# romanwerpachowski/ML

Measured on NVIDIA B200. Metric: em_point_components_per_second, higher is better.
Workload: dtype f64

## Files before the change

### ml_b200/csrc/context.cu

```cuda
#include <dlfcn.h>

#include <algorithm>
#include <cmath>
#include <cstdlib>
#include <cstring>
#include <mutex>
#include <random>
#include <string>
#include <thread>
#include <type_traits>
#include <vector>

#include "internal.h"

namespace mlb {

static thread_local std::string g_last_error = "";

void set_error(const char* fmt, ...)
{
    char buf[1024];
    va_list ap;
    va_start(ap, fmt);
    vsnprintf(buf, sizeof(buf), fmt, ap);
// ... 210 lines not shown
        sum += ms;
    }
    if (total_ms) *total_ms = sum;
    if (launches) *launches = static_cast<int64_t>(used / 2);
    return MLB_OK;
}

void KernelTimer::destroy()
{
    for (cudaEvent_t e : events)
        if (e) cudaEventDestroy(e);
    events.clear();
    used = 0;
}

Layout Layout::make(int64_t n_total)
{
    Layout lay;
    lay.n_total = n_total;
    int64_t c = n_total / (8 * kSmCount * 6);
    c = (c + 127) / 128 * 128;
    c = std::max<int64_t>(128, std::min<int64_t>(2048, c));
    if (const char* env = std::getenv("MLB200_CHUNK")) {
        const long v = std::atol(env);
        if (v >= 128 && v <= 4096 && v % 128 == 0) c = v;
    }
    lay.chunk = static_cast<int>(c);
    lay.n_chunks = (n_total + c - 1) / c;
    for (int v = 0; v <= kVirtualShards; ++v) lay.vshard_chunk[v] = lay.n_chunks * v / kVirtualShards;
    return lay;
}


struct VshardRanges {
    int64_t lo[kVirtualShards];
    int64_t hi[kVirtualShards];
};

__global__ void reduce_partials_kernel(const double* __restrict__ partials, VshardRanges r, int s, double* __restrict__ out)
{
    __shared__ double lanes[8][33];
    const int e = blockIdx.x * 32 + threadIdx.x;
    const int v = blockIdx.y, ty = threadIdx.y;
    double a0 = 0, a1 = 0, a2 = 0, a3 = 0;
    if (e < s) {
        const int64_t hi = r.hi[v];
        for (int64_t c = r.lo[v] + 4 * ty; c < hi; c += 32) {
            a0 += partials[c * s + e];
            if (c + 1 < hi) a1 += partials[(c + 1) * s + e];
            if (c + 2 < hi) a2 += partials[(c + 2) * s + e];
            if (c + 3 < hi) a3 += partials[(c + 3) * s + e];
        }
    }
    lanes[ty][threadIdx.x] = (a0 + a1) + (a2 + a3);
    __syncthreads();
    if (ty == 0 && e < s) {
        const int x = threadIdx.x;
        out[static_cast<int64_t>(v) * s + e] =
            ((lanes[0][x] + lanes[1][x]) + (lanes[2][x] + lanes[3][x])) + ((lanes[4][x] + lanes[5][x]) + (lanes[6][x] + lanes[7][x]));
    }
}

constexpr int kReduceGroup = 32;

__global__ void reduce_groups_kernel(const double* __restrict__ partials, VshardRanges r, int nv, int s, double* __restrict__ out)
{
    __shared__ double lanes[8][33];
    int group = blockIdx.y, v = 0;
    for (; v < nv; ++v) {
        const int ng = static_cast<int>((r.hi[v] - r.lo[v] + kReduceGroup - 1) / kReduceGroup);
        if (group < ng) break;
        group -= ng;
    }
    if (v == nv) return;
    const int64_t lo = r.lo[v] + static_cast<int64_t>(group) * kReduceGroup;
    const int64_t hi = min(lo + kReduceGroup, r.hi[v]);
    const int e = blockIdx.x * 32 + threadIdx.x, ty = threadIdx.y;
    double a0 = 0, a1 = 0, a2 = 0, a3 = 0;
    if (e < s) {
        const int64_t c = lo + 4 * ty;
        if (c < hi) a0 = partials[c * s + e];
        if (c + 1 < hi) a1 = partials[(c + 1) * s + e];
        if (c + 2 < hi) a2 = partials[(c + 2) * s + e];
        if (c + 3 < hi) a3 = partials[(c + 3) * s + e];
    }
    lanes[ty][threadIdx.x] = (a0 + a1) + (a2 + a3);
    __syncthreads();
    if (ty == 0 && e < s) {
        const int x = threadIdx.x;
        out[static_cast<int64_t>(blockIdx.y) * s + e] =
            ((lanes[0][x] + lanes[1][x]) + (lanes[2][x] + lanes[3][x])) + ((lanes[4][x] + lanes[5][x]) + (lanes[6][x] + lanes[7][x]));
    }
}

void ReduceScratch::release(mlb_ctx* ctx)
{
    for (size_t g = 0; g < ptr.size(); ++g)
        if (ptr[g]) {
            cudaSetDevice(ctx->gpus[g].device);
            cudaFreeAsync(ptr[g], ctx->gpus[g].stream);
        }
    ptr.clear();
    len.clear();
}

int reduce_and_exchange_units(mlb_data* data, const std::vector<double*>& partials, const std::vector<double*>& vsum, int s, ReduceScratch& scratch,
                              const int64_t* bounds)
{
    mlb_ctx* ctx = data->ctx;
    const int vpg = ctx->vshards_per_gpu();
    scratch.ptr.resize(ctx->gpus.size(), nullptr);
    scratch.len.resize(ctx->gpus.size(), 0);
    MLB_TRY(for_each_gpu(ctx, [&](int g, Gpu& gpu) -> int {
        const int64_t local_begin = bounds[gpu.rank * vpg];
        VshardRanges r, rg;
        int64_t total_groups = 0;
        for (int j = 0; j < vpg; ++j) {
            const int v = gpu.rank * vpg + j;
            r.lo[j] = bounds[v] - local_begin;
            r.hi[j] = bounds[v + 1] - local_begin;
            rg.lo[j] = total_groups;
            total_groups += (r.hi[j] - r.lo[j] + kReduceGroup - 1) / kReduceGroup;
            rg.hi[j] = total_groups;
        }
        double* out = vsum[g] + static_cast<int64_t>(gpu.rank) * vpg * s;
        if (bounds[kVirtualShards] <= 2 * kReduceGroup * kVirtualShards) {
            reduce_partials_kernel<<<dim3((s + 31) / 32, vpg), dim3(32, 8), 0, gpu.stream>>>(partials[g], r, s, out);
            MLB_CUDA(cudaGetLastError());
            return MLB_OK;
        }
        const size_t need = static_cast<size_t>(total_groups) * s;
        if (scratch.len[g] < need) {
            if (scratch.ptr[g]) {
                MLB_CUDA(cudaFreeAsync(scratch.ptr[g], gpu.stream));
                scratch.ptr[g] = nullptr;
                scratch.len[g] = 0;
            }
            MLB_CUDA(cudaMallocFromPoolAsync(&scratch.ptr[g], sizeof(double) * need, gpu.pool, gpu.stream));
            scratch.len[g] = need;
        }
        reduce_groups_kernel<<<dim3((s + 31) / 32, static_cast<unsigned>(total_groups)), dim3(32, 8), 0, gpu.stream>>>(partials[g], r, vpg, s, scratch.ptr[g]);
        MLB_CUDA(cudaGetLastError());
        reduce_partials_kernel<<<dim3((s + 31) / 32, vpg), dim3(32, 8), 0, gpu.stream>>>(scratch.ptr[g], rg, s, out);
        MLB_CUDA(cudaGetLastError());
        return MLB_OK;
    }));
    if (ctx->world > 1) {
        MLB_NCCL_API(api);
        MLB_NCCL(api, api->GroupStart());
        for (size_t g = 0; g < ctx->gpus.size(); ++g) {
            Gpu& gpu = ctx->gpus[g];
            const size_t count = static_cast<size_t>(vpg) * s;
            MLB_NCCL(api, api->AllGather(vsum[g] + static_cast<int64_t>(gpu.rank) * count, vsum[g], count, ncclDouble, gpu.comm, gpu.stream));
        }
        MLB_NCCL(api, api->GroupEnd());
    }
    return MLB_OK;
}

int reduce_and_exchange(mlb_data* data, const std::vector<double*>& partials, const std::vector<double*>& vsum, int s, ReduceScratch& scratch)
{
    return reduce_and_exchange_units(data, partials, vsum, s, scratch, data->lay.vshard_chunk);
}


__global__ void column_sum_kernel(const double* __restrict__ x, int64_t n_local, int d, int chunk, double* __restrict__ partials)
{
    extern __shared__ double sm[];
    const int64_t p0 = static_cast<int64_t>(blockIdx.x) * chunk;
    const int64_t p1 = min(p0 + chunk, n_local);
    const int lanes = blockDim.x / d;
    const int t = threadIdx.x;
    const int c = t % d, lane = t / d;
    double acc = 0;
    if (lane < lanes) {
        for (int64_t p = p0 + lane; p < p1; p += lanes) acc += x[p * d + c];
    }
    sm[t] = (lane < lanes) ? acc : 0.0;
    __syncthreads();
    if (t < d) {
        double s = 0;
        for (int l = 0; l < lanes; ++l) s += sm[l * d + t];
        partials[static_cast<int64_t>(blockIdx.x) * d + t] = s;
    }
}

static int compute_shift(mlb_data* data)
{
    mlb_ctx* ctx = data->ctx;
    const int d = data->d;
    std::vector<double*> partials(ctx->gpus.size(), nullptr), vsum(ctx->gpus.size(), nullptr);
    MLB_TRY(for_each_gpu(ctx, [&](int g, Gpu& gpu) -> int {
        DataShard& sh = data->shards[g];
        MLB_CUDA(cudaMallocFromPoolAsync(&partials[g], sizeof(double) * std::max<int64_t>(1, sh.n_chunks()) * d, gpu.pool, gpu.stream));
        MLB_CUDA(cudaMallocFromPoolAsync(&vsum[g], sizeof(double) * kVirtualShards * d, gpu.pool, gpu.stream));
// ... 645 lines not shown
```

### ml_b200/csrc/em.cu

```cuda
#include <algorithm>
#include <cmath>
#include <limits>

#include "em_direct.cuh"
#include "em_split.cuh"
#include "fastmath.cuh"
#include "internal.h"

namespace mlb {

constexpr int kTile = 64;
constexpr int kEmThreads = 128;
constexpr int kLogBatch = 16;

__host__ __device__ constexpr int em_ne_offdiag(int DP) { return 4 * (DP / 4) * (DP / 4 - 1) / 2; }
__host__ __device__ constexpr int em_ne(int DP) { return em_ne_offdiag(DP) + 2 * (DP / 4) + (DP / 4 + 1) / 2 + DP / 4; }
__host__ __device__ constexpr int em_estep_offdiag(int DP, int a, int mb)
{
    const int DQ = DP / 4, ma = a / 4, i = a % 4;
    int n = 0;
    for (int m = 0; m < ma; ++m) n += 4 * (DQ - 1 - m);
    return n + i * (DQ - 1 - ma) + (mb - ma - 1);
}
__host__ __device__ constexpr int em_fm_raw(int DP) { return 1 + DP + DP * (DP + 1) / 2; }
__host__ __device__ constexpr int em_nm(int DP) { return (em_fm_raw(DP) + 7) / 8; }
__host__ __device__ constexpr int em_sv(int DP, int KP) { return em_nm(DP) * 8 * KP + 8; }
__host__ __device__ constexpr int em_theta_len(int DP, int KP) { return em_ne(DP) * (KP / 8) * 32 + KP; }

constexpr size_t em_smem_bytes(int DP, int KP)
{
    return sizeof(double) * (em_theta_len(DP, KP) + 2 * kTile * (DP + 4) + kTile * (KP + 4) + 8 + DP + kExpTableSize);
}

struct EmArgs {
    const double* x;
    long long n_local;
    int d, k;
    const double* shift;
    const double* theta;
    const int2* feat_m;
    double* partials;
    int chunk;
    int n_chunks;
    unsigned* counter;
    const double* r_in;
    long long r_ld;
    double* r_out;
    long long r_out_ld;
    unsigned* labels_out;
    long long range_begin, range_count;
};

__device__ __forceinline__ long long min64(long long a, long long b) { return a < b ? a : b; }

__device__ __forceinline__ void dmma(double (&acc)[2], double a, double b)
{
    asm("mma.sync.aligned.m8n8k4.row.col.f64.f64.f64.f64 {%0,%1}, {%2}, {%3}, {%0,%1};" : "+d"(acc[0]), "+d"(acc[1]) : "d"(a), "d"(b));
}

template <int NT>
__device__ __forceinline__ void load_theta_frag(const double* thE, int j, int lane, double (&bf)[NT])
{
    if constexpr (NT == 1) {
        bf[0] = thE[j * 32 + lane];
    } else {
#pragma unroll
        for (int h = 0; h < NT / 2; ++h) {
            const double2 v = reinterpret_cast<const double2*>(thE)[(j * (NT / 2) + h) * 32 + lane];
            bf[2 * h] = v.x;
            bf[2 * h + 1] = v.y;
        }
    }
}

template <int DP, int KP, int MODE>
__global__ void __launch_bounds__(kEmThreads, (DP * KP <= 128 || MODE == 2) ? 4 : 2) em_kernel(const EmArgs p)
{
    constexpr int NT = KP / 8, DQ = DP / 4, NE = em_ne(DP), NM = em_nm(DP);
    constexpr int ZS = DP + 4, RS = KP + 4;
    constexpr int WN = (NM >= 8 || NT == 1) ? 1 : 2, WM = 4 / WN;
    constexpr int MW = (NM + WM - 1) / WM, NW = NT / WN;
    constexpr int SV = em_sv(DP, KP);
    constexpr int XR = kTile * DP / kEmThreads;

    extern __shared__ __align__(16) double sm[];
    double* thE = sm;
    double* cE = thE + NE * NT * 32;
    double* Zb = cE + KP;
    double* R = Zb + 2 * kTile * ZS;
    double* wl = R + kTile * RS;
    double* sh = wl + 8;
    double* etab = sh + DP;
    __shared__ int s_next;

    const int tid = threadIdx.x, lane = tid & 31, warp = tid >> 5, g = lane >> 2, c = lane & 3;
    const int d = p.d;

    if (MODE != 1)
        for (int i = tid; i < em_theta_len(DP, KP); i += kEmThreads) sm[i] = p.theta[i];
    for (int i = tid; i < 2 * kTile * ZS; i += kEmThreads) Zb[i] = 0.0;
    for (int i = tid; i < kTile * RS; i += kEmThreads) R[i] = 0.0;
    if (tid < DP) sh[tid] = tid < d ? p.shift[tid] : 0.0;
    load_exp_table(etab);

    const int wm = warp / WN, wn = warp % WN;
    int ia[MW], ib[MW];
    double sacc[MW][NW][2];
    if (MODE != 2) {
#pragma unroll
        for (int i = 0; i < MW; ++i) {
            const int mt = wm * MW + i;
            const int2 f = mt < NM ? p.feat_m[mt * 8 + g] : make_int2(DP + 1, DP + 1);
            ia[i] = f.x;
            ib[i] = f.y;
        }
    }

    double xr[XR];
    auto load_tile = [&](long long point0, int nvalid) {
        const double* xg = p.x + point0 * d;
        const int nel = nvalid * d;
#pragma unroll
        for (int r = 0; r < XR; ++r) {
            const int e = tid + kEmThreads * r;
            xr[r] = e < nel ? xg[e] : 0.0;
        }
    };
    auto store_tile = [&](double* Z, int nvalid) {
        const int nel = nvalid * d;
#pragma unroll
        for (int r = 0; r < XR; ++r) {
            const int e = tid + kEmThreads * r;
            if (e < kTile * d) {
                const int pt = (d == DP) ? e / DP : FastDiv(d).div(e);
                const int dm = e - pt * d;
                Z[pt * ZS + dm] = e < nel ? xr[r] - sh[dm] : 0.0;
            }
        }
        if (tid < kTile) Z[tid * ZS + DP] = tid < nvalid ? 1.0 : 0.0;
    };

    const long long work_begin = MODE == 2 ? p.range_begin : 0;
    const long long work_end = MODE == 2 ? p.range_begin + p.range_count : p.n_local;

    for (;;) {
        __syncthreads();
        if (tid == 0) s_next = static_cast<int>(atomicAdd(p.counter, 1u));
        __syncthreads();
        const int chunk = s_next;
        if (chunk >= p.n_chunks) break;
        const long long p_begin = work_begin + static_cast<long long>(chunk) * p.chunk;
        const long long p_end = min64(p_begin + p.chunk, work_end);
        const int ntiles = static_cast<int>((p_end - p_begin + kTile - 1) / kTile);

        if (MODE != 2) {
#pragma unroll
            for (int i = 0; i < MW; ++i)
#pragma unroll
                for (int nt = 0; nt < NW; ++nt) sacc[i][nt][0] = sacc[i][nt][1] = 0.0;
        }
        double ll_acc = 0.0, ll_prod = 1.0;

        load_tile(p_begin, static_cast<int>(min64(kTile, p_end - p_begin)));
        store_tile(Zb, static_cast<int>(min64(kTile, p_end - p_begin)));
        __syncthreads();

        for (int t = 0; t < ntiles; ++t) {
            double* Z = Zb + (t & 1) * kTile * ZS;
            const long long tile0 = p_begin + static_cast<long long>(t) * kTile;
            const int nvalid = static_cast<int>(min64(kTile, p_end - tile0));
            const int nvalid_next = t + 1 < ntiles ? static_cast<int>(min64(kTile, p_end - tile0 - kTile)) : 0;
            if (t + 1 < ntiles) load_tile(tile0 + kTile, nvalid_next);

            if (MODE == 1) {
                for (int idx = tid; idx < kTile * p.k; idx += kEmThreads) {
                    const int pt = idx % kTile, kk = idx / kTile;
                    R[pt * RS + kk] = pt < nvalid ? p.r_in[tile0 + pt + kk * p.r_ld] : 0.0;
                }
            } else {
                const double* z0 = Z + (warp * 16 + g) * ZS;
                const double* z1 = z0 + 8 * ZS;
                double acc[2][NT][2];
#pragma unroll
                for (int nt = 0; nt < NT; ++nt) {
                    const double2 cc = *reinterpret_cast<const double2*>(cE + 8 * nt + 2 * c);
                    acc[0][nt][0] = acc[1][nt][0] = cc.x;
                    acc[0][nt][1] = acc[1][nt][1] = cc.y;
                }
                double zc0[DQ], zc1[DQ];
#pragma unroll
                for (int m = 0; m < DQ; ++m) {
                    zc0[m] = z0[4 * m + c];
// ... 28 lines not shown
                    const int o = 4 * mx + c, o2 = 4 * mx + ((c + 2) & 3);
                    const bool live = mx < DQ;
                    const double u0 = live ? z0[o] * z0[o2] : 0.0, u1 = live ? z1[o] * z1[o2] : 0.0;
                    estep(J0 + 2 * DQ + h, u0, u1);
                }
#pragma unroll
                for (int m = 0; m < DQ; ++m) estep(NE - DQ + m, zc0[m], zc1[m]);
                double mxs[2], sums[2];
#pragma unroll
                for (int mt = 0; mt < 2; ++mt) {
                    int mkey = lse_key(acc[mt][0][0]);
#pragma unroll
                    for (int nt = 0; nt < NT; ++nt) mkey = max(mkey, max(lse_key(acc[mt][nt][0]), lse_key(acc[mt][nt][1])));
                    mkey = max(mkey, __shfl_xor_sync(0xffffffffu, mkey, 1));
                    mkey = max(mkey, __shfl_xor_sync(0xffffffffu, mkey, 2));
                    const double mx = lse_shift_of_key(mkey);
                    double sum = 0.0;
#pragma unroll
                    for (int nt = 0; nt < NT; ++nt) {
                        acc[mt][nt][0] = exp_nonpositive(acc[mt][nt][0] - mx, etab);
                        acc[mt][nt][1] = exp_nonpositive(acc[mt][nt][1] - mx, etab);
                        sum += acc[mt][nt][0] + acc[mt][nt][1];
                    }
                    sum += __shfl_xor_sync(0xffffffffu, sum, 1);
                    sum += __shfl_xor_sync(0xffffffffu, sum, 2);
                    mxs[mt] = mx;
                    sums[mt] = sum;
                }
                const double inv_mine = reciprocal_of_sum((c & 1) ? sums[1] : sums[0]);
                const double invs[2] = {__shfl_sync(0xffffffffu, inv_mine, lane & ~1), __shfl_sync(0xffffffffu, inv_mine, lane | 1)};
#pragma unroll
                for (int mt = 0; mt < 2; ++mt) {
                    const int pl = warp * 16 + mt * 8 + g;
                    const double inv = invs[mt];
                    if (c == 0 && pl < nvalid) {
                        ll_acc += mxs[mt];
                        ll_prod *= sums[mt];
                    }
                    if (MODE == 0) {
#pragma unroll
                        for (int nt = 0; nt < NT; ++nt)
                            *reinterpret_cast<double2*>(R + pl * RS + 8 * nt + 2 * c) = make_double2(acc[mt][nt][0] * inv, acc[mt][nt][1] * inv);
                    } else {
                        double best = -1.0;
                        unsigned best_k = 0xffffffffu;
#pragma unroll
                        for (int nt = 0; nt < NT; ++nt)
#pragma unroll
                            for (int e = 0; e < 2; ++e) {
                                const int kk = 8 * nt + 2 * c + e;
                                const double r = acc[mt][nt][e] * inv;
                                if (kk < p.k) {
                                    if (pl < nvalid && p.r_out) p.r_out[(tile0 - p.range_begin) + pl + kk * p.r_out_ld] = r;
                                    if (r > best) { best = r; best_k = kk; }
                                }
                            }
#pragma unroll
                        for (int off = 1; off <= 2; off <<= 1) {
                            const double ob = __shfl_xor_sync(0xffffffffu, best, off);
                            const unsigned ok = __shfl_xor_sync(0xffffffffu, best_k, off);
                            if (ob > best || (ob == best && ok < best_k)) { best = ob; best_k = ok; }
                        }
                        if (c == 0 && pl < nvalid && p.labels_out) p.labels_out[(tile0 - p.range_begin) + pl] = best_k;
                    }
                }
            }
            if (MODE != 2) {
                __syncthreads();
#pragma unroll 4
                for (int s = 0; s < kTile / 4; ++s) {
                    const double* zp = Z + (4 * s + c) * ZS;
                    const double* rp = R + (4 * s + c) * RS + wn * NW * 8 + g;
                    double bf[NW];
#pragma unroll
                    for (int nt = 0; nt < NW; ++nt) bf[nt] = rp[8 * nt];
#pragma unroll
                    for (int i = 0; i < MW; ++i) {
                        if (wm * MW + i < NM) {
                            const double af = zp[ia[i]] * zp[ib[i]];
#pragma unroll
                            for (int nt = 0; nt < NW; ++nt) dmma(sacc[i][nt], af, bf[nt]);
                        }
                    }
                }
            }
            if (MODE != 1 && ((t & (kLogBatch - 1)) == kLogBatch - 1 || t + 1 == ntiles)) {
                ll_acc += log(ll_prod);
                ll_prod = 1.0;
            }
            if (t + 1 < ntiles) store_tile(Zb + ((t + 1) & 1) * kTile * ZS, nvalid_next);
            __syncthreads();
        }

        if (MODE != 2) {
            double* out = p.partials + static_cast<long long>(chunk) * SV;
#pragma unroll
            for (int i = 0; i < MW; ++i) {
                const int mt = wm * MW + i;
                if (mt < NM) {
#pragma unroll
                    for (int nt = 0; nt < NW; ++nt)
                        *reinterpret_cast<double2*>(out + (mt * 8 + g) * KP + (wn * NW + nt) * 8 + 2 * c) = make_double2(sacc[i][nt][0], sacc[i][nt][1]);
                }
            }
#pragma unroll
            for (int off = 16; off >= 1; off >>= 1) ll_acc += __shfl_xor_sync(0xffffffffu, ll_acc, off);
            if (lane == 0) wl[warp] = ll_acc;
            __syncthreads();
            if (tid == 0) out[NM * 8 * KP] = (wl[0] + wl[1]) + (wl[2] + wl[3]);
            if (tid >= 1 && tid < 8) out[NM * 8 * KP + tid] = 0.0;
        }
    }
}

#include "em_small.cuh"

struct EmFinalizeArgs {
    const double* vsum;
    const double* dstats;
    const double* shift;
    int d, k, DP, KP, SV;
    int DPd, dSV;
    long long n_total;
    const int2* feat_m;
    const int2* feat_e;
    int nm8, ne;
    double* means;
    double* covs;
    double* weights;
    double* inv_covs;
    double* sqrt_dets;
    double* theta_out;
    double* dimg_out;
    double* kappa_out;
    int p_in_smem;
    double* ll_ring;
    unsigned long long* ll_counter;
    int ll_ring_len;
};

__global__ void em_finalize_kernel(const EmFinalizeArgs p)
{
    extern __shared__ double fs[];
// ... 171 lines not shown
    __shared__ double etab[kExpTableSize];
    load_exp_table(etab);
    __syncthreads();
    const long long i = static_cast<long long>(blockIdx.x) * blockDim.x + threadIdx.x;
    if (i < n) out[i] = exp_nonpositive(x[i], etab);
}


using EmKernelFn = void (*)(EmArgs);

template <int MODE>
static EmKernelFn em_kernel_for(int DP, int KP)
{
#define EM_CASE(D_, K_) if (DP == D_ && KP == K_) return em_kernel<D_, K_, MODE>;
#define EM_SMALL_CASE(D_, K_) if (DP == D_ && KP == K_) return em_small_kernel<D_, K_, MODE>;
    EM_SMALL_CASE(4, 8) EM_SMALL_CASE(4, 16) EM_SMALL_CASE(4, 32)
    EM_SMALL_CASE(8, 8) EM_SMALL_CASE(8, 16) EM_SMALL_CASE(8, 32)
    EM_CASE(16, 8) EM_CASE(16, 16) EM_CASE(16, 32)
#undef EM_CASE
#undef EM_SMALL_CASE
    return nullptr;
}

struct EmGpu {
    double* theta[2] = {nullptr, nullptr};
    double* params = nullptr;
    double* partials = nullptr;
    double* vsum = nullptr;
    double* ll = nullptr;
    unsigned long long* ll_counter = nullptr;
    int2* feat_m = nullptr;
    int2* feat_e = nullptr;
    unsigned* counter = nullptr;
    double* stage = nullptr;
    unsigned* stage_labels = nullptr;
    int grid = 0;
    double* r = nullptr;
    double* ll_tile = nullptr;
    int2* feat_e_off = nullptr;
    int grid_e = 0, grid_m = 0;
    KernelTimer timer;
};

using EmSplitKernelFn = void (*)(EmSplitArgs);

struct EmDirectGpu {
    double* img = nullptr;
    double* kappa = nullptr;
    double* r = nullptr;
    double* ll_tile = nullptr;
    double* partials = nullptr;
    double* vsum = nullptr;
    long long* sc_begin = nullptr;
    int2* tile_tab = nullptr;
    int n_sc = 0;
    int grid_e = 0, grid_m = 0;
};

struct EmDirect {
    bool capable = false;
    bool ready = false;
    int DP = 0, NB = 0, KPr = 0, IMG = 0, L = 0, SVd = 0;
    int cb = 1, cg = 1, tiles_per_range = 0, n_ranges = 1;
    size_t smem_e = 0, smem_m = 0;
    int64_t sc_bounds[kVirtualShards + 1] = {};
    std::vector<EmDirectGpu> gpus;
// ... 9 lines not shown
}

using namespace mlb;

struct mlb_em {
    mlb_ctx* ctx = nullptr;
    mlb_data* data = nullptr;
    int d = 0, k = 0, DP = 0, KP = 0, NT = 0, NE = 0, NM = 0, SV = 0;
    std::vector<int2> feat_m, feat_e;
    std::vector<EmGpu> gpus;
    int cur = 0;
    bool have_params = false, have_step = false;
    int last_path = 0;
    int64_t direct_steps = 0;
    int64_t launches = 0;
    int64_t steps_done = 0;
    EmKernelFn fn_step = nullptr, fn_mstep = nullptr, fn_emit = nullptr;
    int path = 1;
    EmDirect dr;
    int forced_path = 0;
    int route = 1;
    double kappa_max = 0.0;
    bool r_direct_valid = false;
    double* kappa_host = nullptr;
    EmSplitKernelFn fn_split_e = nullptr, fn_split_m = nullptr;
    size_t smem_split_e = 0, smem_split_m = 0;
    size_t smem_fused = 0;
    int MW = 4;
    cudaGraphExec_t step_graph[2] = {nullptr, nullptr};
    int64_t launches_per_step = 0;
    int plain_steps = 0;
    ReduceScratch reduce_scratch;

    double* means(int g) const { return gpus[g].params; }
    double* covs(int g) const { return gpus[g].params + d * k; }
    double* weights(int g) const { return covs(g) + static_cast<size_t>(k) * d * d; }
    double* inv_covs(int g) const { return weights(g) + k; }
    double* sqrt_dets(int g) const { return inv_covs(g) + static_cast<size_t>(k) * d * d; }
    size_t params_len() const { return static_cast<size_t>(d) * k + 2 * static_cast<size_t>(k) * d * d + 2 * k; }
};

namespace mlb {

static int pad_to(int v, const int* options, int n)
{
    for (int i = 0; i < n; ++i)
        if (v <= options[i]) return options[i];
    return 0;
}

static EmArgs base_args(const mlb_em* em, int g)
{
    const DataShard& sh = em->data->shards[g];
    const EmGpu& eg = em->gpus[g];
    EmArgs a{};
    a.x = sh.x;
    a.n_local = sh.n();
    a.d = em->d;
    a.k = em->k;
    a.shift = sh.shift;
    a.theta = eg.theta[em->cur];
    a.feat_m = eg.feat_m;
    a.partials = eg.partials;
    a.chunk = em->data->lay.chunk;
    a.n_chunks = static_cast<int>(sh.n_chunks());
    a.counter = eg.counter;
    return a;
}

static int launch_em(mlb_em* em, EmKernelFn fn, const EmArgs& a, int g, int grid)
{
    Gpu& gpu = em->ctx->gpus[g];
    MLB_CUDA(cudaMemsetAsync(a.counter, 0, sizeof(unsigned), gpu.stream));
    if (a.n_chunks > 0) {
        const bool timed = fn == em->fn_step;
        if (timed) MLB_TRY(em->gpus[g].timer.begin(gpu.stream));
        fn<<<std::min(grid, a.n_chunks), em->DP <= 8 ? kSmallThreads : kEmThreads, em->smem_fused, gpu.stream>>>(a);
        MLB_CUDA(cudaGetLastError());
        if (timed) MLB_TRY(em->gpus[g].timer.end(gpu.stream));
        ++em->launches;
    }
    return MLB_OK;
}

static EmSplitArgs split_args(const mlb_em* em, int g, const double* theta)
{
    const DataShard& sh = em->data->shards[g];
    const EmGpu& eg = em->gpus[g];
    EmSplitArgs a{};
    a.x = sh.x;
    a.n_local = sh.n();
    a.d = em->d; a.k = em->k; a.DP = em->DP; a.KP = em->KP;
    a.shift = sh.shift;
    a.theta = theta;
    a.feat_e = eg.feat_e_off;
    a.feat_m = eg.feat_m;
    a.ne = em->NE; a.nm = em->NM;
    a.r = eg.r;
    a.partials = eg.partials;
    a.ll_tile = eg.ll_tile;
    a.sv = em->SV;
    a.chunk = em->data->lay.chunk;
    a.n_chunks = static_cast<int>(sh.n_chunks());
    a.counter = eg.counter;
    return a;
}
// ... 234 lines not shown
    MLB_CUDA(cudaMemcpyAsync(em->kappa_host, em->dr.gpus[0].kappa, sizeof(double) * em->k, cudaMemcpyDeviceToHost, gpu.stream));
    return MLB_OK;
}

static void route_finish(mlb_em* em)
{
    em->kappa_max = 0.0;
    if (em->dr.capable && em->kappa_host)
        for (int i = 0; i < em->k; ++i) {
            const double v = em->kappa_host[i];
            if (v != v) em->kappa_max = std::numeric_limits<double>::infinity();
            else if (v > em->kappa_max) em->kappa_max = v;
        }
    const bool direct = em->path == 0 || em->forced_path == 3 || (em->dr.capable && em->kappa_max > kKappaDirect);
    em->route = direct ? 3 : em->path;
}

static int update_route(mlb_em* em)
{
    MLB_TRY(route_enqueue(em));
    MLB_CUDA(cudaStreamSynchronize(em->ctx->gpus[0].stream));
    route_finish(em);
    return MLB_OK;
}

static int enqueue_step_plain(mlb_em* em)
{
    mlb_ctx* ctx = em->ctx;
    MLB_TRY(for_each_gpu(ctx, [&](int g, Gpu&) -> int {
        return launch_pass(em, g, em->gpus[g].theta[em->cur], true);
    }));
    std::vector<double*> partials, vsum;
    for (EmGpu& eg : em->gpus) { partials.push_back(eg.partials); vsum.push_back(eg.vsum); }
    MLB_TRY(reduce_and_exchange(em->data, partials, vsum, em->SV, em->reduce_scratch));
    em->launches += static_cast<int64_t>(ctx->gpus.size());
    MLB_TRY(for_each_gpu(ctx, [&](int g, Gpu&) -> int {
        return launch_finalize(em, g, 1, em->cur ^ 1, true);
    }));
    em->r_direct_valid = false;
    return MLB_OK;
}

static int enqueue_step(mlb_em* em)
{
    mlb_ctx* ctx = em->ctx;
    if (em->route == 3) {
        MLB_TRY(enqueue_step_direct(em));
        em->cur ^= 1;
        em->last_path = 3;
        ++em->direct_steps;
        return MLB_OK;
    }
    em->last_path = em->path;
    const bool graphable = ctx->gpus.size() == 1 && ctx->world == 1 && !em->gpus[0].timer.enabled && em->plain_steps >= 2;
    if (!graphable) {
        MLB_TRY(enqueue_step_plain(em));
        ++em->plain_steps;
        em->cur ^= 1;
        return MLB_OK;
    }
    Gpu& gpu = ctx->gpus[0];
    MLB_CUDA(cudaSetDevice(gpu.device));
    cudaGraphExec_t& exec = em->step_graph[em->cur];
    if (!exec) {
        const int64_t launches_before = em->launches;
        cudaGraph_t graph = nullptr;
        MLB_CUDA(cudaStreamBeginCapture(gpu.stream, cudaStreamCaptureModeThreadLocal));
// ... 50 lines not shown
        const int64_t n = em->data->shards[g].n();
        if (n == 0) return MLB_OK;
        const long long total = static_cast<long long>(n) * em->dr.KPr;
        em_split_import_r_kernel<<<static_cast<unsigned>((total + 255) / 256), 256, 0, gpu.stream>>>(dev[g], n, n, em->k, em->dr.KPr, em->dr.gpus[g].r);
        MLB_CUDA(cudaGetLastError());
        ++em->launches;
        return MLB_OK;
    });
}

static int mstep_from_device(mlb_em* em, std::vector<double*>& dev, int rc)
{
    mlb_ctx* ctx = em->ctx;
    auto body = [&]() -> int {
        const bool direct_only = em->path == 0 || em->forced_path == 3;
        if (!direct_only) {
            MLB_TRY(for_each_gpu(ctx, [&](int g, Gpu&) -> int {
                const int64_t n = em->data->shards[g].n();
                if (em->path == 2) {
                    if (n == 0) return MLB_OK;
                    const long long total = static_cast<long long>(n) * em->KP;
                    em_split_import_r_kernel<<<static_cast<unsigned>((total + 255) / 256), 256, 0, ctx->gpus[g].stream>>>(dev[g], n, n, em->k, em->KP, em->gpus[g].r);
                    MLB_CUDA(cudaGetLastError());
                    ++em->launches;
                    return launch_split(em, g, em->gpus[g].theta[em->cur], false, false);
                }
                EmArgs a = base_args(em, g);
                a.r_in = dev[g];
                a.r_ld = std::max<int64_t>(1, n);
                return launch_em(em, em->fn_mstep, a, g, em->gpus[g].grid);
            }));
            std::vector<double*> partials, vsum;
            for (EmGpu& eg : em->gpus) { partials.push_back(eg.partials); vsum.push_back(eg.vsum); }
            MLB_TRY(reduce_and_exchange(em->data, partials, vsum, em->SV, em->reduce_scratch));
            em->launches += static_cast<int64_t>(ctx->gpus.size());
            MLB_TRY(for_each_gpu(ctx, [&](int g, Gpu&) -> int { return launch_finalize(em, g, 1, em->cur, false); }));
            MLB_TRY(update_route(em));
            if (em->route != 3) return MLB_OK;
        }
        MLB_TRY(direct_prepare(em));
        MLB_TRY(direct_import_r(em, dev));
        MLB_TRY(direct_mstep_from_r(em, direct_only));
        return update_route(em);
    };
    if (rc == MLB_OK) rc = body();
    const int rc_sync = mlb_ctx_synchronize(ctx);
    if (rc == MLB_OK) rc = rc_sync;
    for (size_t g = 0; g < dev.size(); ++g)
        if (dev[g]) { cudaSetDevice(ctx->gpus[g].device); cudaFreeAsync(dev[g], ctx->gpus[g].stream); }
    if (rc == MLB_OK) { em->have_params = true; em->have_step = false; }
    return rc;
}

static int direct_sample_covariance(mlb_em* em, double* cov_out)
{
    MLB_TRY(direct_prepare(em));
    mlb_ctx* ctx = em->ctx;
    EmDirect& dr = em->dr;
    const int d = em->d;
    std::vector<double*> tmp(ctx->gpus.size(), nullptr);
    int rc = for_each_gpu(ctx, [&](int g, Gpu& gpu) -> int {
        MLB_CUDA(cudaMallocFromPoolAsync(&tmp[g], sizeof(double) * dr.IMG, gpu.pool, gpu.stream));
        MLB_CUDA(cudaMemsetAsync(tmp[g], 0, sizeof(double) * dr.IMG, gpu.stream));
        EmDirectArgs a = direct_args(em, g);
        a.img = tmp[g];
        a.k = 1;
        a.unit_r = 1;
// ... 146 lines not shown
        dr.IMG = dr_img_len(dr.DP);
        dr.L = dr_stat_len(dr.DP);
        const long long svd = static_cast<long long>(k) * dr.L + 8;
        if (svd >= (1ll << 31)) { delete em; set_error("mlb_em_create: D=%d, K=%d: statistics vector too long", data->d, k); return MLB_EINVAL; }
        dr.SVd = static_cast<int>(svd);
        dr.cb = static_cast<int>(std::max<size_t>(1, std::min<size_t>(std::min(16, k), (12 * 1024) / (sizeof(double) * dr.IMG))));
        const int T = dr_tiles(dr.NB);
        if (T <= 4 * kDrSlots) {
            const int by_smem = static_cast<int>((96 * 1024) / (sizeof(double) * 2 * kDrSub * (dr.DP + 12))) - 1;
            dr.cg = std::max(1, std::min({16, k, 4 * kDrSlots / T, by_smem}));
            dr.tiles_per_range = T;
            dr.n_ranges = 1;
        } else {
            dr.cg = 1;
            dr.tiles_per_range = 4 * kDrSlots;
            dr.n_ranges = (T + 4 * kDrSlots - 1) / (4 * kDrSlots);
        }
        dr.smem_e = em_direct_e_smem(dr.DP, dr.cb);
        dr.smem_m = em_direct_m_smem(dr.DP, dr.cg, em->d);
        dr.sc_bounds[0] = 0;
        for (int v = 0; v < kVirtualShards; ++v)
            dr.sc_bounds[v + 1] = dr.sc_bounds[v] + std::min<int64_t>(data->lay.vshard_chunk[v + 1] - data->lay.vshard_chunk[v], kDrSuperPerVshard);
        dr.gpus.resize(ctx->gpus.size());
    }
    em->gpus.resize(ctx->gpus.size());
    int rc = for_each_gpu(ctx, [&](int g, Gpu& gpu) -> int {
        EmGpu& eg = em->gpus[g];
        EmDirectGpu& dg = em->dr.gpus[g];
        const DataShard& sh = data->shards[g];
        MLB_CUDA(cudaMallocFromPoolAsync(&eg.params, sizeof(double) * em->params_len(), gpu.pool, gpu.stream));
        MLB_CUDA(cudaMallocFromPoolAsync(&eg.ll, sizeof(double) * kLlRing, gpu.pool, gpu.stream));
        MLB_CUDA(cudaMallocFromPoolAsync(&eg.ll_counter, sizeof(unsigned long long), gpu.pool, gpu.stream));
        MLB_CUDA(cudaMemsetAsync(eg.ll_counter, 0, sizeof(unsigned long long), gpu.stream));
        MLB_CUDA(cudaMallocFromPoolAsync(&eg.counter, sizeof(unsigned), gpu.pool, gpu.stream));
        MLB_CUDA(cudaMallocFromPoolAsync(&dg.img, sizeof(double) * static_cast<size_t>(k) * em->dr.IMG, gpu.pool, gpu.stream));
        MLB_CUDA(cudaMallocFromPoolAsync(&dg.kappa, sizeof(double) * k, gpu.pool, gpu.stream));
        MLB_CUDA(cudaMemsetAsync(dg.kappa, 0, sizeof(double) * k, gpu.stream));
        {
            const size_t fin_smem = finalize_smem(em, nullptr);
            if (fin_smem > 48 * 1024)
                MLB_CUDA(cudaFuncSetAttribute(reinterpret_cast<const void*>(em_finalize_kernel), cudaFuncAttributeMaxDynamicSharedMemorySize, static_cast<int>(fin_smem)));
        }
        int sms = 0;
        MLB_CUDA(cudaDeviceGetAttribute(&sms, cudaDevAttrMultiProcessorCount, gpu.device));
        if (em->path) {
            const size_t theta_len = static_cast<size_t>(em_theta_len(DP, KP));
            MLB_CUDA(cudaMallocFromPoolAsync(&eg.theta[0], sizeof(double) * theta_len, gpu.pool, gpu.stream));
            MLB_CUDA(cudaMallocFromPoolAsync(&eg.theta[1], sizeof(double) * theta_len, gpu.pool, gpu.stream));
            MLB_CUDA(cudaMallocFromPoolAsync(&eg.partials, sizeof(double) * std::max<int64_t>(1, sh.n_chunks()) * em->SV, gpu.pool, gpu.stream));
            MLB_CUDA(cudaMallocFromPoolAsync(&eg.vsum, sizeof(double) * kVirtualShards * em->SV, gpu.pool, gpu.stream));
            MLB_CUDA(cudaMallocFromPoolAsync(&eg.feat_m, sizeof(int2) * em->feat_m.size(), gpu.pool, gpu.stream));
            MLB_CUDA(cudaMallocFromPoolAsync(&eg.feat_e, sizeof(int2) * em->feat_e.size(), gpu.pool, gpu.stream));
            MLB_CUDA(cudaMemsetAsync(eg.vsum, 0, sizeof(double) * kVirtualShards * em->SV, gpu.stream));
            MLB_CUDA(cudaMemcpyAsync(eg.feat_m, em->feat_m.data(), sizeof(int2) * em->feat_m.size(), cudaMemcpyHostToDevice, gpu.stream));
            MLB_CUDA(cudaMemcpyAsync(eg.feat_e, em->feat_e.data(), sizeof(int2) * em->feat_e.size(), cudaMemcpyHostToDevice, gpu.stream));
        }
        if (em->path == 1) {
            const size_t smem = em->smem_fused;
            for (EmKernelFn fn : {em->fn_step, em->fn_mstep, em->fn_emit})
                MLB_CUDA(cudaFuncSetAttribute(reinterpret_cast<const void*>(fn), cudaFuncAttributeMaxDynamicSharedMemorySize, static_cast<int>(smem)));
            int per_sm = 0;
            MLB_CUDA(cudaOccupancyMaxActiveBlocksPerMultiprocessor(&per_sm, reinterpret_cast<const void*>(em->fn_step), em->DP <= 8 ? kSmallThreads : kEmThreads, smem));
            MLB_REQUIRE(per_sm >= 1, "mlb_em_create: EM kernel does not fit on an SM");
            eg.grid = per_sm * sms;
        } else if (em->path == 2) {
            std::vector<int2> off(em->feat_e.size());
            for (size_t i = 0; i < off.size(); ++i) off[i] = em->feat_e[i].x < 0 ? make_int2(DP + 1, DP + 1) : em->feat_e[i];
// ... 500 lines not shown
```

### ml_b200/csrc/internal.h

```cpp
#pragma once

#include <cuda_runtime.h>
#include <nccl.h>

#include <cstdarg>
#include <cstdint>
#include <cstdio>
#include <mutex>
#include <string>
#include <vector>

#include "../../include/mlb200.h"

namespace mlb {

void set_error(const char* fmt, ...);

#define MLB_CUDA(expr)                                                                          \
    do {                                                                                        \
        cudaError_t mlb_e_ = (expr);                                                            \
        if (mlb_e_ != cudaSuccess) {                                                            \
            ::mlb::set_error("%s:%d: %s failed: %s", __FILE__, __LINE__, #expr, cudaGetErrorString(mlb_e_)); \
            return (mlb_e_ == cudaErrorMemoryAllocation) ? MLB_ENOMEM : MLB_ECUDA;              \
        }                                                                                       \
// ... 99 lines not shown
    int64_t n() const { return end - begin; }
    int64_t n_chunks() const { return chunk_end - chunk_begin; }
};

}

struct mlb_data {
    mlb_ctx* ctx = nullptr;
    mlb::Layout lay;
    int d = 0;
    std::vector<mlb::DataShard> shards;
    std::vector<double> shift;
    int64_t launches = 0;
};

namespace mlb {

struct DeviceRestore {
    int saved = -1;
    DeviceRestore() { if (cudaGetDevice(&saved) != cudaSuccess) { saved = -1; cudaGetLastError(); } }
    ~DeviceRestore() { if (saved >= 0) cudaSetDevice(saved); }
};

template <class F>
int for_each_gpu(mlb_ctx* ctx, F&& body)
{
    for (size_t g = 0; g < ctx->gpus.size(); ++g) {
        MLB_CUDA(cudaSetDevice(ctx->gpus[g].device));
        MLB_TRY(body(static_cast<int>(g), ctx->gpus[g]));
    }
    return MLB_OK;
}

struct ReduceScratch {
    std::vector<double*> ptr;
    std::vector<size_t> len;
    void release(mlb_ctx* ctx);
};

int reduce_and_exchange(mlb_data* data, const std::vector<double*>& partials, const std::vector<double*>& vsum, int s, ReduceScratch& scratch);
int reduce_and_exchange_units(mlb_data* data, const std::vector<double*>& partials, const std::vector<double*>& vsum, int s, ReduceScratch& scratch,
                              const int64_t* bounds);

int staged_h2d(Gpu& gpu, void* dst_device, const void* src, size_t rows, size_t row_bytes, size_t src_stride);
int staged_d2h(Gpu& gpu, void* dst, const void* src_device, size_t bytes);
int staged_d2h_2d(Gpu& gpu, void* dst, size_t dst_stride, const void* src_device, size_t src_stride, size_t rows, size_t row_bytes);

struct KernelTimer {
    bool enabled = false;
    std::vector<cudaEvent_t> events;
    size_t used = 0;
    static constexpr size_t kMaxLaunches = 4096;
    int begin(cudaStream_t stream);
    int end(cudaStream_t stream);
    int total(double* total_ms, int64_t* launches);
    void reset() { used = 0; }
    void destroy();
};

__host__ __device__ inline double tree8(const double* v, int64_t stride)
{
    return ((v[0] + v[stride]) + (v[2 * stride] + v[3 * stride])) + ((v[4 * stride] + v[5 * stride]) + (v[6 * stride] + v[7 * stride]));
}

}
```

Before: 48.56.

## Fold first-level group reduction into EM kernel and specialize D=16,K=32 accumulation

For the D=16, K=32 path, the EM step kernel now uses a count-row-aware split of second-moment tile work across warps. This drops redundant MMA tiles and writes the count row directly from a warp shuffle reduction. Each block also atomically counts arrivals per 32-chunk group, and the last block to arrive sums that group's partials into a scratch buffer. This lets the host skip the separate reduce_groups_kernel launch and its extra pass over partials. The cost is threadfences, atomics and a serialized tail reduction in the final block of each group, plus a specialized indexing scheme that only holds for one shape.

```diff
diff --git a/ml_b200/csrc/context.cu b/ml_b200/csrc/context.cu
--- a/ml_b200/csrc/context.cu
+++ b/ml_b200/csrc/context.cu
@@ -266,11 +266,6 @@
 }
 
 
-struct VshardRanges {
-    int64_t lo[kVirtualShards];
-    int64_t hi[kVirtualShards];
-};
-
 __global__ void reduce_partials_kernel(const double* __restrict__ partials, VshardRanges r, int s, double* __restrict__ out)
 {
     __shared__ double lanes[8][33];
@@ -295,8 +290,6 @@
     }
 }
 
-constexpr int kReduceGroup = 32;
-
 __global__ void reduce_groups_kernel(const double* __restrict__ partials, VshardRanges r, int nv, int s, double* __restrict__ out)
 {
     __shared__ double lanes[8][33];
@@ -310,21 +303,43 @@
     const int64_t lo = r.lo[v] + static_cast<int64_t>(group) * kReduceGroup;
     const int64_t hi = min(lo + kReduceGroup, r.hi[v]);
     const int e = blockIdx.x * 32 + threadIdx.x, ty = threadIdx.y;
-    double a0 = 0, a1 = 0, a2 = 0, a3 = 0;
-    if (e < s) {
-        const int64_t c = lo + 4 * ty;
-        if (c < hi) a0 = partials[c * s + e];
-        if (c + 1 < hi) a1 = partials[(c + 1) * s + e];
-        if (c + 2 < hi) a2 = partials[(c + 2) * s + e];
-        if (c + 3 < hi) a3 = partials[(c + 3) * s + e];
-    }
-    lanes[ty][threadIdx.x] = (a0 + a1) + (a2 + a3);
+    lanes[ty][threadIdx.x] = e < s ? group_lane(partials, lo, hi, s, e, ty) : 0.0;
     __syncthreads();
-    if (ty == 0 && e < s) {
-        const int x = threadIdx.x;
-        out[static_cast<int64_t>(blockIdx.y) * s + e] =
-            ((lanes[0][x] + lanes[1][x]) + (lanes[2][x] + lanes[3][x])) + ((lanes[4][x] + lanes[5][x]) + (lanes[6][x] + lanes[7][x]));
-    }
+    if (ty == 0 && e < s) out[static_cast<int64_t>(blockIdx.y) * s + e] = tree8(&lanes[0][threadIdx.x], 33);
+}
+
+ChunkGroups chunk_groups(const mlb_ctx* ctx, const Gpu& gpu, const int64_t* bounds)
+{
+    ChunkGroups cg;
+    cg.nv = ctx->vshards_per_gpu();
+    const int64_t local_begin = bounds[gpu.rank * cg.nv];
+    int64_t total_groups = 0;
+    for (int j = 0; j < cg.nv; ++j) {
+        const int v = gpu.rank * cg.nv + j;
+        cg.r.lo[j] = bounds[v] - local_begin;
+        cg.r.hi[j] = bounds[v + 1] - local_begin;
+        cg.rg.lo[j] = total_groups;
+        total_groups += (cg.r.hi[j] - cg.r.lo[j] + kReduceGroup - 1) / kReduceGroup;
+        cg.rg.hi[j] = total_groups;
+    }
+    cg.two_level = bounds[kVirtualShards] > 2 * kReduceGroup * kVirtualShards;
+    return cg;
+}
+
+int reserve_group_sums(mlb_ctx* ctx, int g, size_t need, ReduceScratch& scratch)
+{
+    scratch.ptr.resize(ctx->gpus.size(), nullptr);
+    scratch.len.resize(ctx->gpus.size(), 0);
+    if (scratch.len[g] >= need) return MLB_OK;
+    Gpu& gpu = ctx->gpus[g];
+    if (scratch.ptr[g]) {
+        MLB_CUDA(cudaFreeAsync(scratch.ptr[g], gpu.stream));
+        scratch.ptr[g] = nullptr;
+        scratch.len[g] = 0;
+    }
+    MLB_CUDA(cudaMallocFromPoolAsync(&scratch.ptr[g], sizeof(double) * need, gpu.pool, gpu.stream));
+    scratch.len[g] = need;
+    return MLB_OK;
 }
 
 void ReduceScratch::release(mlb_ctx* ctx)
@@ -339,43 +354,25 @@
 }
 
 int reduce_and_exchange_units(mlb_data* data, const std::vector<double*>& partials, const std::vector<double*>& vsum, int s, ReduceScratch& scratch,
-                              const int64_t* bounds)
+                              const int64_t* bounds, bool groups_folded)
 {
     mlb_ctx* ctx = data->ctx;
     const int vpg = ctx->vshards_per_gpu();
-    scratch.ptr.resize(ctx->gpus.size(), nullptr);
-    scratch.len.resize(ctx->gpus.size(), 0);
     MLB_TRY(for_each_gpu(ctx, [&](int g, Gpu& gpu) -> int {
-        const int64_t local_begin = bounds[gpu.rank * vpg];
-        VshardRanges r, rg;
-        int64_t total_groups = 0;
-        for (int j = 0; j < vpg; ++j) {
-            const int v = gpu.rank * vpg + j;
-            r.lo[j] = bounds[v] - local_begin;
-            r.hi[j] = bounds[v + 1] - local_begin;
-            rg.lo[j] = total_groups;
-            total_groups += (r.hi[j] - r.lo[j] + kReduceGroup - 1) / kReduceGroup;
-            rg.hi[j] = total_groups;
-        }
+        const ChunkGroups cg = chunk_groups(ctx, gpu, bounds);
         double* out = vsum[g] + static_cast<int64_t>(gpu.rank) * vpg * s;
-        if (bounds[kVirtualShards] <= 2 * kReduceGroup * kVirtualShards) {
-            reduce_partials_kernel<<<dim3((s + 31) / 32, vpg), dim3(32, 8), 0, gpu.stream>>>(partials[g], r, s, out);
+        if (!cg.two_level) {
+            reduce_partials_kernel<<<dim3((s + 31) / 32, vpg), dim3(32, 8), 0, gpu.stream>>>(partials[g], cg.r, s, out);
             MLB_CUDA(cudaGetLastError());
             return MLB_OK;
         }
-        const size_t need = static_cast<size_t>(total_groups) * s;
-        if (scratch.len[g] < need) {
-            if (scratch.ptr[g]) {
-                MLB_CUDA(cudaFreeAsync(scratch.ptr[g], gpu.stream));
-                scratch.ptr[g] = nullptr;
-                scratch.len[g] = 0;
-            }
-            MLB_CUDA(cudaMallocFromPoolAsync(&scratch.ptr[g], sizeof(double) * need, gpu.pool, gpu.stream));
-            scratch.len[g] = need;
-        }
-        reduce_groups_kernel<<<dim3((s + 31) / 32, static_cast<unsigned>(total_groups)), dim3(32, 8), 0, gpu.stream>>>(partials[g], r, vpg, s, scratch.ptr[g]);
-        MLB_CUDA(cudaGetLastError());
-        reduce_partials_kernel<<<dim3((s + 31) / 32, vpg), dim3(32, 8), 0, gpu.stream>>>(scratch.ptr[g], rg, s, out);
+        MLB_TRY(reserve_group_sums(ctx, g, static_cast<size_t>(cg.groups()) * s, scratch));
+        if (!groups_folded) {
+            reduce_groups_kernel<<<dim3((s + 31) / 32, static_cast<unsigned>(cg.groups())), dim3(32, 8), 0, gpu.stream>>>(partials[g], cg.r, vpg, s,
+                                                                                                                        scratch.ptr[g]);
+            MLB_CUDA(cudaGetLastError());
+        }
+        reduce_partials_kernel<<<dim3((s + 31) / 32, vpg), dim3(32, 8), 0, gpu.stream>>>(scratch.ptr[g], cg.rg, s, out);
         MLB_CUDA(cudaGetLastError());
         return MLB_OK;
     }));
@@ -392,9 +389,10 @@
     return MLB_OK;
 }
 
-int reduce_and_exchange(mlb_data* data, const std::vector<double*>& partials, const std::vector<double*>& vsum, int s, ReduceScratch& scratch)
-{
-    return reduce_and_exchange_units(data, partials, vsum, s, scratch, data->lay.vshard_chunk);
+int reduce_and_exchange(mlb_data* data, const std::vector<double*>& partials, const std::vector<double*>& vsum, int s, ReduceScratch& scratch,
+                        bool groups_folded)
+{
+    return reduce_and_exchange_units(data, partials, vsum, s, scratch, data->lay.vshard_chunk, groups_folded);
 }
 
 
diff --git a/ml_b200/csrc/em.cu b/ml_b200/csrc/em.cu
--- a/ml_b200/csrc/em.cu
+++ b/ml_b200/csrc/em.cu
@@ -43,6 +43,9 @@
     int chunk;
     int n_chunks;
     unsigned* counter;
+    double* groups;
+    unsigned* arrivals;
+    ChunkGroups cg;
     const double* r_in;
     long long r_ld;
     double* r_out;
@@ -82,6 +85,8 @@
     constexpr int MW = (NM + WM - 1) / WM, NW = NT / WN;
     constexpr int SV = em_sv(DP, KP);
     constexpr int XR = kTile * DP / kEmThreads;
+    constexpr bool CF = DP == 16 && KP == 32 && MODE != 2;
+    static_assert(!CF || (em_fm_raw(DP) - 1 == 19 * 8 && NM == 20 && WN == 1 && NW == 4), "count-row split assumes D = 16, K = 32");
 
     extern __shared__ __align__(16) double sm[];
     double* thE = sm;
@@ -104,9 +109,19 @@
     load_exp_table(etab);
 
     const int wm = warp / WN, wn = warp % WN;
-    int ia[MW], ib[MW];
+    constexpr int MF = CF ? 6 : MW;
+    int ia[MF], ib[MF];
     double sacc[MW][NW][2];
-    if (MODE != 2) {
+    double cnt = 0.0;
+    if constexpr (CF) {
+#pragma unroll
+        for (int i = 0; i < MF; ++i) {
+            const int ft = i < 4 ? 4 * warp + i : 16 + (3 * warp + 2 * (i - 4)) / 4;
+            const int2 f = p.feat_m[1 + ft * 8 + g];
+            ia[i] = f.x;
+            ib[i] = f.y;
+        }
+    } else if (MODE != 2) {
 #pragma unroll
         for (int i = 0; i < MW; ++i) {
             const int mt = wm * MW + i;
@@ -158,6 +173,7 @@
             for (int i = 0; i < MW; ++i)
 #pragma unroll
                 for (int nt = 0; nt < NW; ++nt) sacc[i][nt][0] = sacc[i][nt][1] = 0.0;
+            cnt = 0.0;
         }
         double ll_acc = 0.0, ll_prod = 1.0;
 
@@ -252,7 +268,7 @@
 #pragma unroll
                 for (int mt = 0; mt < 2; ++mt) {
                     const int pl = warp * 16 + mt * 8 + g;
-                    const double inv = invs[mt];
+                    const double inv = CF && pl >= nvalid ? 0.0 : invs[mt];
                     if (c == 0 && pl < nvalid) {
                         ll_acc += mxs[mt];
                         ll_prod *= sums[mt];
@@ -285,7 +301,29 @@
                     }
                 }
             }
-            if (MODE != 2) {
+            if constexpr (CF) {
+                __syncthreads();
+                const double* rb = R + c * RS + g;
+                const bool u1_hi = (3 * warp + 1) / 4 != 3 * warp / 4;
+                const int ct0 = 8 * ((3 * warp) & 3), ct1 = 8 * ((3 * warp + 1) & 3), ct2 = 8 * ((3 * warp + 2) & 3), ct3 = 8 * ((3 * warp + 3) & 3);
+#pragma unroll 4
+                for (int s = 0; s < kTile / 4; ++s) {
+                    const double* zp = Z + (4 * s + c) * ZS;
+                    const double* rp = rb + 4 * s * RS;
+                    const double bf[4] = {rp[ct0], rp[ct1], rp[ct2], rp[ct3]};
+                    cnt += bf[0];
+#pragma unroll
+                    for (int i = 0; i < 4; ++i) {
+                        const double af = zp[ia[i]] * zp[ib[i]];
+#pragma unroll
+                        for (int j = 0; j < 4; ++j) dmma(sacc[i][j], af, bf[j]);
+                    }
+                    const double ax0 = zp[ia[4]] * zp[ib[4]], ax1 = zp[ia[5]] * zp[ib[5]];
+                    dmma(sacc[4][0], ax0, bf[0]);
+                    dmma(sacc[4][1], u1_hi ? ax1 : ax0, bf[1]);
+                    dmma(sacc[4][2], ax1, bf[2]);
+                }
+            } else if (MODE != 2) {
                 __syncthreads();
 #pragma unroll 4
                 for (int s = 0; s < kTile / 4; ++s) {
@@ -314,13 +352,29 @@
 
         if (MODE != 2) {
             double* out = p.partials + static_cast<long long>(chunk) * SV;
-#pragma unroll
-            for (int i = 0; i < MW; ++i) {
-                const int mt = wm * MW + i;
-                if (mt < NM) {
-#pragma unroll
-                    for (int nt = 0; nt < NW; ++nt)
-                        *reinterpret_cast<double2*>(out + (mt * 8 + g) * KP + (wn * NW + nt) * 8 + 2 * c) = make_double2(sacc[i][nt][0], sacc[i][nt][1]);
+            if constexpr (CF) {
+                auto put = [&](int ft, int ct, const double (&v)[2]) {
+                    *reinterpret_cast<double2*>(out + (1 + ft * 8 + g) * KP + ct * 8 + 2 * c) = make_double2(v[0], v[1]);
+                };
+#pragma unroll
+                for (int i = 0; i < 4; ++i)
+#pragma unroll
+                    for (int j = 0; j < 4; ++j) put(4 * warp + i, (3 * warp + j) & 3, sacc[i][j]);
+#pragma unroll
+                for (int u = 0; u < 3; ++u) put(16 + (3 * warp + u) / 4, (3 * warp + u) & 3, sacc[4][u]);
+                cnt += __shfl_xor_sync(0xffffffffu, cnt, 1);
+                cnt += __shfl_xor_sync(0xffffffffu, cnt, 2);
+                if (c == 0) out[((3 * warp) & 3) * 8 + g] = cnt;
+                for (int e = tid; e < (NM * 8 - em_fm_raw(DP)) * KP; e += kEmThreads) out[em_fm_raw(DP) * KP + e] = 0.0;
+            } else {
+#pragma unroll
+                for (int i = 0; i < MW; ++i) {
+                    const int mt = wm * MW + i;
+                    if (mt < NM) {
+#pragma unroll
+                        for (int nt = 0; nt < NW; ++nt)
+                            *reinterpret_cast<double2*>(out + (mt * 8 + g) * KP + (wn * NW + nt) * 8 + 2 * c) = make_double2(sacc[i][nt][0], sacc[i][nt][1]);
+                    }
                 }
             }
 #pragma unroll
@@ -329,6 +383,36 @@
             __syncthreads();
             if (tid == 0) out[NM * 8 * KP] = (wl[0] + wl[1]) + (wl[2] + wl[3]);
             if (tid >= 1 && tid < 8) out[NM * 8 * KP + tid] = 0.0;
+            if (p.groups) {
+                auto group_of = [&](long long& lo, long long& hi) {
+                    int j = 0;
+                    while (chunk >= p.cg.r.hi[j]) ++j;
+                    const long long gi = (chunk - p.cg.r.lo[j]) / kReduceGroup;
+                    lo = p.cg.r.lo[j] + gi * kReduceGroup;
+                    hi = min64(lo + kReduceGroup, p.cg.r.hi[j]);
+                    return p.cg.rg.lo[j] + gi;
+                };
+                __threadfence();
+                __syncthreads();
+                if (tid == 0) {
+                    long long lo, hi;
+                    const long long group = group_of(lo, hi);
+                    s_next = atomicAdd(p.arrivals + group, 1u) == static_cast<unsigned>(hi - lo - 1);
+                }
+                __syncthreads();
+                if (s_next) {
+                    __threadfence();
+                    long long lo, hi;
+                    double* gs = p.groups + group_of(lo, hi) * SV;
+#pragma unroll 2
+                    for (int e = tid; e < SV; e += kEmThreads) {
+                        double lanes[8];
+#pragma unroll
+                        for (int l = 0; l < 8; ++l) lanes[l] = group_lane(p.partials, lo, hi, SV, e, l);
+                        gs[e] = tree8(lanes, 1);
+                    }
+                }
+            }
         }
     }
 }
@@ -566,6 +650,7 @@
     int2* feat_m = nullptr;
     int2* feat_e = nullptr;
     unsigned* counter = nullptr;
+    ChunkGroups groups;
     double* stage = nullptr;
     unsigned* stage_labels = nullptr;
     int grid = 0;
@@ -641,6 +726,8 @@
     int plain_steps = 0;
     ReduceScratch reduce_scratch;
 
+    bool folds_groups() const { return path == 1 && DP == 16; }
+
     double* means(int g) const { return gpus[g].params; }
     double* covs(int g) const { return gpus[g].params + d * k; }
     double* weights(int g) const { return covs(g) + static_cast<size_t>(k) * d * d; }
@@ -677,10 +764,18 @@
     return a;
 }
 
-static int launch_em(mlb_em* em, EmKernelFn fn, const EmArgs& a, int g, int grid)
+static int launch_em(mlb_em* em, EmKernelFn fn, EmArgs a, int g, int grid)
 {
     Gpu& gpu = em->ctx->gpus[g];
-    MLB_CUDA(cudaMemsetAsync(a.counter, 0, sizeof(unsigned), gpu.stream));
+    const ChunkGroups& cg = em->gpus[g].groups;
+    const bool fold = fn != em->fn_emit && em->folds_groups() && cg.two_level;
+    MLB_CUDA(cudaMemsetAsync(a.counter, 0, sizeof(unsigned) * (fold ? 1 + cg.groups() : 1), gpu.stream));
+    if (fold) {
+        MLB_TRY(reserve_group_sums(em->ctx, g, static_cast<size_t>(cg.groups()) * em->SV, em->reduce_scratch));
+        a.groups = em->reduce_scratch.ptr[g];
+        a.arrivals = a.counter + 1;
+        a.cg = cg;
+    }
     if (a.n_chunks > 0) {
         const bool timed = fn == em->fn_step;
         if (timed) MLB_TRY(em->gpus[g].timer.begin(gpu.stream));
@@ -981,7 +1076,7 @@
     }));
     std::vector<double*> partials, vsum;
     for (EmGpu& eg : em->gpus) { partials.push_back(eg.partials); vsum.push_back(eg.vsum); }
-    MLB_TRY(reduce_and_exchange(em->data, partials, vsum, em->SV, em->reduce_scratch));
+    MLB_TRY(reduce_and_exchange(em->data, partials, vsum, em->SV, em->reduce_scratch, em->folds_groups()));
     em->launches += static_cast<int64_t>(ctx->gpus.size());
     MLB_TRY(for_each_gpu(ctx, [&](int g, Gpu&) -> int {
         return launch_finalize(em, g, 1, em->cur ^ 1, true);
@@ -1098,7 +1193,7 @@
             }));
             std::vector<double*> partials, vsum;
             for (EmGpu& eg : em->gpus) { partials.push_back(eg.partials); vsum.push_back(eg.vsum); }
-            MLB_TRY(reduce_and_exchange(em->data, partials, vsum, em->SV, em->reduce_scratch));
+            MLB_TRY(reduce_and_exchange(em->data, partials, vsum, em->SV, em->reduce_scratch, em->folds_groups()));
             em->launches += static_cast<int64_t>(ctx->gpus.size());
             MLB_TRY(for_each_gpu(ctx, [&](int g, Gpu&) -> int { return launch_finalize(em, g, 1, em->cur, false); }));
             MLB_TRY(update_route(em));
@@ -1311,7 +1406,8 @@
         MLB_CUDA(cudaMallocFromPoolAsync(&eg.ll, sizeof(double) * kLlRing, gpu.pool, gpu.stream));
         MLB_CUDA(cudaMallocFromPoolAsync(&eg.ll_counter, sizeof(unsigned long long), gpu.pool, gpu.stream));
         MLB_CUDA(cudaMemsetAsync(eg.ll_counter, 0, sizeof(unsigned long long), gpu.stream));
-        MLB_CUDA(cudaMallocFromPoolAsync(&eg.counter, sizeof(unsigned), gpu.pool, gpu.stream));
+        eg.groups = chunk_groups(ctx, gpu, data->lay.vshard_chunk);
+        MLB_CUDA(cudaMallocFromPoolAsync(&eg.counter, sizeof(unsigned) * (1 + eg.groups.groups()), gpu.pool, gpu.stream));
         MLB_CUDA(cudaMallocFromPoolAsync(&dg.img, sizeof(double) * static_cast<size_t>(k) * em->dr.IMG, gpu.pool, gpu.stream));
         MLB_CUDA(cudaMallocFromPoolAsync(&dg.kappa, sizeof(double) * k, gpu.pool, gpu.stream));
         MLB_CUDA(cudaMemsetAsync(dg.kappa, 0, sizeof(double) * k, gpu.stream));
diff --git a/ml_b200/csrc/internal.h b/ml_b200/csrc/internal.h
--- a/ml_b200/csrc/internal.h
+++ b/ml_b200/csrc/internal.h
@@ -155,15 +155,42 @@
     return MLB_OK;
 }
 
+constexpr int kReduceGroup = 32;
+
+struct VshardRanges {
+    int64_t lo[kVirtualShards];
+    int64_t hi[kVirtualShards];
+};
+
+struct ChunkGroups {
+    VshardRanges r, rg;
+    int nv = 0;
+    bool two_level = false;
+    int64_t groups() const { return nv ? rg.hi[nv - 1] : 0; }
+};
+ChunkGroups chunk_groups(const mlb_ctx* ctx, const Gpu& gpu, const int64_t* bounds);
+
+__device__ __forceinline__ double group_lane(const double* partials, int64_t lo, int64_t hi, int s, int e, int l)
+{
+    const int64_t c = lo + 4 * l;
+    const double a0 = c < hi ? __ldcg(partials + c * s + e) : 0.0;
+    const double a1 = c + 1 < hi ? __ldcg(partials + (c + 1) * s + e) : 0.0;
+    const double a2 = c + 2 < hi ? __ldcg(partials + (c + 2) * s + e) : 0.0;
+    const double a3 = c + 3 < hi ? __ldcg(partials + (c + 3) * s + e) : 0.0;
+    return (a0 + a1) + (a2 + a3);
+}
+
 struct ReduceScratch {
     std::vector<double*> ptr;
     std::vector<size_t> len;
     void release(mlb_ctx* ctx);
 };
 
-int reduce_and_exchange(mlb_data* data, const std::vector<double*>& partials, const std::vector<double*>& vsum, int s, ReduceScratch& scratch);
+int reduce_and_exchange(mlb_data* data, const std::vector<double*>& partials, const std::vector<double*>& vsum, int s, ReduceScratch& scratch,
+                        bool groups_folded = false);
 int reduce_and_exchange_units(mlb_data* data, const std::vector<double*>& partials, const std::vector<double*>& vsum, int s, ReduceScratch& scratch,
-                              const int64_t* bounds);
+                              const int64_t* bounds, bool groups_folded = false);
+int reserve_group_sums(mlb_ctx* ctx, int g, size_t need, ReduceScratch& scratch);
 
 int staged_h2d(Gpu& gpu, void* dst_device, const void* src, size_t rows, size_t row_bytes, size_t src_stride);
 int staged_d2h(Gpu& gpu, void* dst, const void* src_device, size_t bytes);
```

New measurement: 49.39 (median of 6 runs). 1.02x the previous value.
